# CCIG-Champalimaud/adell-mri

Hardware: AMD Instinct MI355X
Metric: volumes/sec 3D U-Net 128^3 2-ch seg (train step: fwd+loss+bwd+SGD) (higher is better)
Workload: dtype f32 (f16x3 split MFMA, fp32 accumulate); 1 GPU; BASELINE configs[1]: u-net-3d-resnet.yaml UNetPL, 2x128^3, batch 2/GPU, dice+focal, SGD-Nesterov; per_gpu_batch=2, parallelism=dp1, yaml=configs/u-net-3d-resnet.yaml, built_by=parse_config_unet -> get_segmentation_network('unet'), gradient_exchange=none (1 rank)

## Files before the change

### adell_mri_amd/_lib.py

```python
import ctypes
import os

_HERE = os.path.dirname(os.path.abspath(__file__))
LIB_PATH = os.environ.get("ADELL_HIP_LIBRARY") or os.path.join(_HERE, "libadellhip.so")

_lib = None

OK = 0
E_BADARG, E_UNSUPPORTED, E_HIP, E_NOMEM = -1, -2, -3, -4

ACT_IDS = {
    "identity": 0, "swish": 1, "silu": 1, "relu": 2, "leaky_relu": 3, "prelu": 4,
    "gelu": 5, "sigmoid": 6, "tanh": 7, "elu": 8,
}


class AdellHipError(RuntimeError):
    pass


class ConvDesc(ctypes.Structure):
    _fields_ = [(n, ctypes.c_int32) for n in (
        "N", "D", "H", "W", "C0", "C1", "Cout", "KD", "KH", "KW", "SD", "SH", "SW",
        "PD", "PH", "PW", "Do", "Ho", "Wo")]
# ... 213 lines not shown
    "adell_gather_nd": (_i, [_vp, _vp, _i, _vp, _vp, _vp, _i, _vp, _vp, _vp, _vp]),
    "adell_layernorm_rows_fwd": (_i, [_vp, _l, _i, _i, _l, _l, _vp, _vp, _f, _vp, _vp, _vp, _vp]),
    "adell_layernorm_rows_bwd_workspace": (_l, [_l, _i]),
    "adell_layernorm_rows_bwd": (_i, [_vp, _vp, _vp, _vp, _vp, _l, _i, _i, _l, _l, _vp, _l, _l,
                                      _vp, _vp, _vp, ctypes.c_size_t, _vp]),
    "adell_winattn_fwd": (_i, [_vp, _vp, _vp, _l, _l, _vp, _vp, _i, _l, _i, _i, _i, _i, _f, _f,
                               ctypes.c_ulong, ctypes.c_uint, _vp, _vp, _vp]),
    "adell_winattn_bwd": (_i, [_vp, _vp, _vp, _l, _l, _vp, _vp, _i, _vp, _vp, _vp, _l, _i, _i, _i,
                               _i, _f, _f, ctypes.c_ulong, ctypes.c_uint, _vp, _vp, _vp, _vp, _vp]),
    "adell_gemm_f32_workspace_floats": (_l, [_i, _i, _i]),
    "adell_gemm_f32": (_i, [_i, _i, _i, _vp, _l, _i, _vp, _l, _i, _vp, _l, _vp, _vp, _l, _vp, _vp]),
    "adell_absmax_f32": (_i, [_vp, _l, _vp, _vp]),
    "adell_gemm_f16x3_applicable": (_i, [_i, _i, _i, _vp, _l, _i, _vp, _l, _i]),
    "adell_gemm_f16x3_workspace_floats": (_l, [_i, _i, _i]),
    "adell_gemm_f16x3": (_i, [_i, _i, _i, _vp, _l, _i, _vp, _l, _i, _vp, _l, _vp, _vp, _l, _vp, _vp,
                              _vp, _vp]),
    "adell_gemm_f16x3_act": (_i, [_i, _i, _i, _vp, _l, _i, _vp, _l, _i, _vp, _l, _vp, _vp, _l, _vp,
                                  _vp, _vp, _i, _f, _vp, _vp, _vp]),
    "adell_optim_step": (_i, [_i, _vp, _vp, _vp, _vp, _l, _f, _f, _f, ctypes.POINTER(ctypes.c_float),
                              _vp]),
    "adell_seg_loss_workspace": (_l, [_i, _l, _i]),
    "adell_seg_loss_fwd": (_i, [_i, _vp, _vp, _vp, _i, _l, _i, _f, _f, _f, _f, _f, _f, _vp, _vp, _vp,
                                ctypes.c_size_t, _vp]),
    "adell_seg_loss_bwd": (_i, [_i, _vp, _vp, _vp, _i, _l, _i, _f, _f, _f, _f, _f, _f, _vp, _vp, _vp,
                                _vp]),
    "adell_channel_softmax_fwd": (_i, [_vp, _vp, _l, _i, _vp]),
    "adell_channel_softmax_bwd": (_i, [_vp, _vp, _vp, _l, _i, _vp]),
    "adell_channel_max_fwd": (_i, [_vp, _vp, _vp, _i, _l, _i, _vp]),
    "adell_channel_max_bwd": (_i, [_vp, _vp, _vp, _i, _l, _i, _vp]),
    "adell_debug_force_conv_cfg": (None, [_i]),
    "adell_set_tuning": (_i, [ctypes.c_char_p, _i]),
    "adell_rng_advance": (_i, [ctypes.c_uint32, _i, _vp]),
    "adell_get_tuning": (_i, [ctypes.c_char_p]),
}


def lib():
    global _lib
    if _lib is None:
        if not os.path.exists(LIB_PATH):
            raise AdellHipError(
                f"{LIB_PATH} not found: build it with `python -c 'import __graft_entry__ as g; "
                "g.build()'` (or `make -C adell_mri_amd/csrc`). adell_mri_amd has no fallback path."
            )
        import torch

        h = ctypes.CDLL(LIB_PATH)
        for name, (res, args) in SIGNATURES.items():
            fn = getattr(h, name)
            fn.restype = res
            fn.argtypes = args
        _lib = h
    return _lib


def check(rc):
    if rc != OK:
        msg = lib().adell_last_error().decode("utf-8", "replace")
        kind = {E_BADARG: "bad argument", E_UNSUPPORTED: "unsupported", E_HIP: "HIP error",
                E_NOMEM: "out of memory"}.get(rc, f"error {rc}")
        raise AdellHipError(f"libadellhip: {kind}: {msg}")
    return rc


class tuning:

# ... 17 lines not shown
```

### adell_mri_amd/csrc/api.hip

```cpp
#include "common.h"
#include <stdarg.h>

static thread_local char g_err[512] = "";

void adell_set_error(const char* fmt, ...) {
  va_list ap;
  va_start(ap, fmt);
  vsnprintf(g_err, sizeof(g_err), fmt, ap);
  va_end(ap);
}

extern "C" const char* adell_last_error(void) { return g_err; }
extern "C" int adell_abi_version(void) { return ADELL_ABI_VERSION; }

int adell_cu_count() {
  static const int cus = [] {
    int dev = 0, n = 0;
    if (hipGetDevice(&dev) != hipSuccess ||
        hipDeviceGetAttribute(&n, hipDeviceAttributeMultiprocessorCount, dev) != hipSuccess)
      n = 0;
    return n > 0 ? n : 256;
  }();
  return cus;
}

#include <stdlib.h>
#include <string.h>

static int adell_env_int(const char* name, int dflt) {
  const char* v = getenv(name);
  return v ? atoi(v) : dflt;
}
static int adell_env_set(const char* name) { return getenv(name) != nullptr; }

static AdellTuning adell_tuning_from_env() {
  AdellTuning t;
  t.igemm_nospec = adell_env_set("ADELL_IGEMM_NOSPEC");
  t.igemm_no8 = adell_env_set("ADELL_IGEMM_NO8");
  t.no_splitk = adell_env_set("ADELL_NO_SPLITK");
  t.wgrad_nozring = adell_env_set("ADELL_WGRAD_NOZRING");
  t.attn_nomfma = adell_env_set("ADELL_ATTN_NOMFMA");
  t.dw_nomfma = adell_env_int("ADELL_DW_NOMFMA", 0);
  t.dw_wgrad_nomfma = adell_env_int("ADELL_DW_WGRAD_NOMFMA", 0);
  t.wgrad_no16 = adell_env_int("ADELL_WGRAD_NO16", 0);
  t.igemm_no16 = adell_env_int("ADELL_IGEMM_NO16", 0);
  t.gemm_norows = adell_env_int("ADELL_GEMM_NOROWS", 0);
#ifdef ADELL_DEBUG
  t.igemm_dbg = adell_env_int("ADELL_IGEMM_DBG", 0);
  t.zr_dbg = adell_env_int("ADELL_ZR_DBG", 0);
#else
  t.igemm_dbg = 0;
  t.zr_dbg = 0;
#endif
  return t;
}
AdellTuning g_adell_tune = adell_tuning_from_env();
long g_adell_plan_epoch = 0;
extern "C" long adell_plan_epoch(void) { return g_adell_plan_epoch; }

static int* adell_tuning_slot(const char* name) {
  if (!name) return nullptr;
  if (!strcmp(name, "igemm_nospec")) return &g_adell_tune.igemm_nospec;
  if (!strcmp(name, "igemm_no8")) return &g_adell_tune.igemm_no8;
  if (!strcmp(name, "no_splitk")) return &g_adell_tune.no_splitk;
  if (!strcmp(name, "wgrad_nozring")) return &g_adell_tune.wgrad_nozring;
  if (!strcmp(name, "attn_nomfma")) return &g_adell_tune.attn_nomfma;
  if (!strcmp(name, "dw_nomfma")) return &g_adell_tune.dw_nomfma;
  if (!strcmp(name, "dw_wgrad_nomfma")) return &g_adell_tune.dw_wgrad_nomfma;
  if (!strcmp(name, "wgrad_no16")) return &g_adell_tune.wgrad_no16;
  if (!strcmp(name, "igemm_no16")) return &g_adell_tune.igemm_no16;
  if (!strcmp(name, "gemm_norows")) return &g_adell_tune.gemm_norows;
#ifdef ADELL_DEBUG
  if (!strcmp(name, "igemm_dbg")) return &g_adell_tune.igemm_dbg;
  if (!strcmp(name, "zr_dbg")) return &g_adell_tune.zr_dbg;
#endif
  return nullptr;
}

extern "C" int adell_set_tuning(const char* name, int value) {
  int* slot = adell_tuning_slot(name);
  if (!slot) {
    adell_set_error("adell_set_tuning: unknown switch '%s'", name ? name : "(null)");
    return ADELL_E_BADARG;
  }
  if (*slot != value) ++g_adell_plan_epoch;
  *slot = value;
  return ADELL_OK;
}

extern "C" int adell_get_tuning(const char* name) {
  int* slot = adell_tuning_slot(name);
  return slot ? *slot : -1;
}

int adell_rng_advance_norm_act(unsigned delta, int set, hipStream_t st);
int adell_rng_advance_tokens(unsigned delta, int set, hipStream_t st);
int adell_rng_advance_window(unsigned delta, int set, hipStream_t st);

extern "C" int adell_rng_advance(uint32_t delta, int set, void* stream) {
  hipStream_t st = (hipStream_t)stream;
  int rc = adell_rng_advance_norm_act(delta, set, st);
  if (rc == ADELL_OK) rc = adell_rng_advance_tokens(delta, set, st);
  if (rc == ADELL_OK) rc = adell_rng_advance_window(delta, set, st);
  if (rc != ADELL_OK) adell_set_error("adell_rng_advance: launch failed");
// ... 3 lines not shown
```

### adell_mri_amd/csrc/common.h

```cpp
#pragma once
#include <hip/hip_runtime.h>
#include <stdint.h>
#include <stdio.h>
#include "../../include/adell_hip.h"

typedef float f32x16 __attribute__((ext_vector_type(16)));
typedef float f32x4 __attribute__((ext_vector_type(4)));

#define ADELL_WAVE 64
#define ADELL_GLOBAL __attribute__((address_space(1)))

void adell_set_error(const char* fmt, ...);

struct AdellTuning {
  int igemm_nospec;
  int igemm_no8;
  int no_splitk;
  int wgrad_nozring;
  int attn_nomfma;
  int dw_nomfma;
  int dw_wgrad_nomfma;
  int wgrad_no16;
  int igemm_no16;
  int gemm_norows;
  int igemm_dbg, zr_dbg;
};
extern AdellTuning g_adell_tune;
extern long g_adell_plan_epoch;
#define ADELL_REQUIRE_ROWS(ptr, have, need, what)                                              \
  ADELL_REQUIRE((ptr) == nullptr || (long)(have) == (long)(need),                              \
                "%s: partial-sum buffer sized for %ld rows per item, the current launch plan "  \
                "writes %ld (query the matching *_ntiles again after adell_set_tuning)",        \
                what, (long)(have), (long)(need))
#ifdef ADELL_DEBUG
#define ADELL_DBG(bits) (bits)
#else
#define ADELL_DBG(bits) 0
#endif

#define ADELL_CHECK_HIP(expr)                                                  \
  do {                                                                         \
    hipError_t _e = (expr);                                                    \
    if (_e != hipSuccess) {                                                    \
      adell_set_error("%s:%d: %s -> %s", __FILE__, __LINE__, #expr,            \
                      hipGetErrorString(_e));                                  \
      return ADELL_E_HIP;                                                      \
    }                                                                          \
  } while (0)

#define ADELL_REQUIRE(cond, ...)                                               \
  do {                                                                         \
    if (!(cond)) {                                                             \
      adell_set_error(__VA_ARGS__);                                            \
      return ADELL_E_BADARG;                                                   \
    }                                                                          \
  } while (0)

// ... 121 lines not shown
```

### adell_mri_amd/csrc/norm_act.hip

```cpp
#include "common.h"

ADELL_RNG_STEP_DEFINE(norm_act)

__global__ __launch_bounds__(256) void adell_stats_finalize_kernel(
    const float* __restrict__ part, int N, int ntiles, int C, double count, float eps,
    int per_item, float* __restrict__ mean, float* __restrict__ rstd) {
  __shared__ double sh[8][32][2];
  const int cl = threadIdx.x & 31, sl = threadIdx.x >> 5;
  const int c = blockIdx.x * 32 + cl;
  const int nbeg = per_item ? blockIdx.y : 0, nend = per_item ? blockIdx.y + 1 : N;
  double s1 = 0.0, s2 = 0.0;
  if (c < C) {
    for (int n = nbeg; n < nend; ++n) {
      const float* p = part + ((size_t)n * ntiles * C + c) * 2;
      int t = sl;
      for (; t + 56 < ntiles; t += 64) {
        float2 v[8];
#pragma unroll
        for (int u = 0; u < 8; ++u)
          v[u] = *reinterpret_cast<const float2*>(p + (size_t)(t + 8 * u) * C * 2);
#pragma unroll
        for (int u = 0; u < 8; ++u) {
          s1 += (double)v[u].x;
          s2 += (double)v[u].y;
        }
      }
      for (; t < ntiles; t += 8) {
        const float2 v = *reinterpret_cast<const float2*>(p + (size_t)t * C * 2);
        s1 += (double)v.x;
        s2 += (double)v.y;
      }
    }
  }
  sh[sl][cl][0] = s1;
  sh[sl][cl][1] = s2;
  __syncthreads();
  if (sl == 0 && c < C) {
    double a = 0.0, b = 0.0;
#pragma unroll
    for (int k = 0; k < 8; ++k) {
      a += sh[k][cl][0];
      b += sh[k][cl][1];
    }
    const double cnt = per_item ? count : count * N;
    const double m = a / cnt;
    double var = b / cnt - m * m;
    if (var < 0.0) var = 0.0;
    const size_t o = per_item ? (size_t)blockIdx.y * C + c : (size_t)c;
    mean[o] = (float)m;
    rstd[o] = (float)(1.0 / sqrt(var + (double)eps));
  }
}

__global__ __launch_bounds__(256) void adell_stats_fold_kernel(const float* __restrict__ part,
                                                               int ntiles, int C, int Z,
                                                               float* __restrict__ out,
                                                               int pstride, int poff) {
  __shared__ double sh[8][32][2];
  const int cl = threadIdx.x & 31, sl = threadIdx.x >> 5;
  const int c = blockIdx.x * 32 + cl, n = blockIdx.y, z = blockIdx.z;
  const int t0 = z * 256;
  const int t1 = t0 + 256 < ntiles ? t0 + 256 : ntiles;
  double s1 = 0.0, s2 = 0.0;
  if (c < C) {
    const float* p = part + ((size_t)n * ntiles * pstride + poff + c) * 2;
    int t = t0 + sl;
    for (; t + 56 < t1; t += 64) {
      float2 v[8];
#pragma unroll
      for (int u = 0; u < 8; ++u)
        v[u] = *reinterpret_cast<const float2*>(p + (size_t)(t + 8 * u) * pstride * 2);
#pragma unroll
      for (int u = 0; u < 8; ++u) {
        s1 += (double)v[u].x;
        s2 += (double)v[u].y;
      }
    }
    for (; t < t1; t += 8) {
      const float2 v = *reinterpret_cast<const float2*>(p + (size_t)t * pstride * 2);
      s1 += (double)v.x;
      s2 += (double)v.y;
    }
  }
  sh[sl][cl][0] = s1;
  sh[sl][cl][1] = s2;
  __syncthreads();
  if (sl == 0 && c < C) {
    double a = 0.0, b = 0.0;
#pragma unroll
    for (int k = 0; k < 8; ++k) {
      a += sh[k][cl][0];
      b += sh[k][cl][1];
    }
    float* o = out + (((size_t)n * Z + z) * C + c) * 2;
    o[0] = (float)a;
    o[1] = (float)b;
  }
}

extern "C" long adell_stats_finalize_workspace(int N, int ntiles, int C) {
  if (ntiles <= 512) return 0;
  const long Z = (ntiles + 255) / 256;
  return (long)sizeof(float) * N * Z * C * 2;
}

extern "C" int adell_stats_finalize(const float* partials, int N, int ntiles, int C,
                                    long count, float eps, int per_item, float* mean,
                                    float* rstd, void* workspace, size_t workspace_bytes,
                                    void* stream) {
  ADELL_REQUIRE(partials && mean && rstd, "stats_finalize: null pointer");
  ADELL_REQUIRE(N > 0 && ntiles > 0 && C > 0 && count > 0, "stats_finalize: bad dims");
  hipStream_t st = (hipStream_t)stream;
  const long need = adell_stats_finalize_workspace(N, ntiles, C);
  if (need > 0) {
    ADELL_REQUIRE(workspace && (long)workspace_bytes >= need,
                  "stats_finalize: workspace too small");
    const int Z = (ntiles + 255) / 256;
    hipLaunchKernelGGL(adell_stats_fold_kernel, dim3(adell_cdiv(C, 32), N, Z), dim3(256), 0, st,
                       partials, ntiles, C, Z, (float*)workspace, C, 0);
    partials = (const float*)workspace;
    ntiles = Z;
  }
  hipLaunchKernelGGL(adell_stats_finalize_kernel, dim3(adell_cdiv(C, 32), per_item ? N : 1),
                     dim3(256), 0, st, partials, N, ntiles, C, (double)count, eps, per_item, mean,
                     rstd);
  ADELL_CHECK_HIP(hipGetLastError());
  return ADELL_OK;
}

__global__ __launch_bounds__(256) void adell_bn_running_update_kernel(
    const float* __restrict__ mean, const float* __restrict__ rstd, float* __restrict__ rmean,
    float* __restrict__ rvar, long long* __restrict__ nbt, int C, float unbias, float eps,
    float momentum) {
  long long t = nbt != nullptr ? nbt[0] + 1 : 0;
  const float mom = momentum >= 0.f ? momentum : 1.f / (float)t;
  __syncthreads();
  for (int c = threadIdx.x; c < C; c += 256) {
    const float r = rstd[c];
    const float var = (1.f / (r * r) - eps) * unbias;
    rmean[c] = rmean[c] * (1.f - mom) + mom * mean[c];
    rvar[c] = rvar[c] * (1.f - mom) + mom * var;
  }
  if (threadIdx.x == 0 && nbt != nullptr) nbt[0] = t;
}

extern "C" int adell_bn_running_update(const float* mean, const float* rstd, float* running_mean,
                                       float* running_var, long long* num_batches_tracked, int C,
                                       long count, float eps, float momentum, void* stream) {
  ADELL_REQUIRE(mean && rstd && running_mean && running_var && C > 0 && count > 0,
                "bn_running_update: bad arguments");
  ADELL_REQUIRE(momentum >= 0.f || num_batches_tracked != nullptr,
                "bn_running_update: the cumulative average needs num_batches_tracked");
  const float unbias = (float)((double)count / (double)(count > 1 ? count - 1 : 1));
  hipLaunchKernelGGL(adell_bn_running_update_kernel, dim3(1), dim3(256), 0, (hipStream_t)stream, mean,
                     rstd, running_mean, running_var, num_batches_tracked, C, unbias, eps, momentum);
// ... 575 lines not shown
    if (sl == 0 && c < C) {
      double A = 0.0, B = 0.0;
#pragma unroll
      for (int k = 0; k < 32; ++k) {
        A += sh[k][cl][0];
        B += sh[k][cl][1];
      }
      accA += A;
      accB += B;
      if (per_item) {
        const double g = gamma ? (double)gamma[c] : 1.0;
        c1[(size_t)n * C + c] = (float)(g * A / count);
        c2[(size_t)n * C + c] = (float)(g * B / count);
      }
    }
    __syncthreads();
  }
  if (sl == 0 && c < C) {
    if (!per_item) {
      const double g = gamma ? (double)gamma[c] : 1.0;
      c1[c] = (float)(g * accA / (count * N));
      c2[c] = (float)(g * accB / (count * N));
    }
    if (dgamma) dgamma[c] = (float)accB;
    if (dbeta) dbeta[c] = (float)accA;
  }
}

__global__ __launch_bounds__(256) void adell_na_bwd_finalize_item_kernel(
    const float* __restrict__ part, int ntiles, int C, double count,
    const float* __restrict__ gamma, float* __restrict__ c1, float* __restrict__ c2,
    int pstride, int poff) {
  __shared__ double sh[32][8][2];
  const int cl = threadIdx.x & 7, sl = threadIdx.x >> 3;
  const int c = blockIdx.x * 8 + cl, n = blockIdx.y;
  double a0 = 0.0, a1 = 0.0, b0 = 0.0, b1 = 0.0;
  if (c < C) {
    int t = sl;
    for (; t + 32 < ntiles; t += 64) {
      const float2 u =
          *reinterpret_cast<const float2*>(part + (((size_t)n * ntiles + t) * pstride + poff + c) * 2);
      const float2 v = *reinterpret_cast<const float2*>(
          part + (((size_t)n * ntiles + t + 32) * pstride + poff + c) * 2);
      a0 += (double)u.x; b0 += (double)u.y;
      a1 += (double)v.x; b1 += (double)v.y;
    }
    for (; t < ntiles; t += 32) {
      const float2 u =
          *reinterpret_cast<const float2*>(part + (((size_t)n * ntiles + t) * pstride + poff + c) * 2);
      a0 += (double)u.x; b0 += (double)u.y;
    }
  }
  sh[sl][cl][0] = a0 + a1;
  sh[sl][cl][1] = b0 + b1;
  __syncthreads();
  if (sl == 0 && c < C) {
    double A = 0.0, B = 0.0;
#pragma unroll
    for (int k = 0; k < 32; ++k) {
      A += sh[k][cl][0];
      B += sh[k][cl][1];
    }
    const double g = gamma ? (double)gamma[c] : 1.0;
    c1[(size_t)n * C + c] = (float)(g * A / count);
    c2[(size_t)n * C + c] = (float)(g * B / count);
  }
}

template <bool VEC>
__global__ __launch_bounds__(256) void adell_na_bwd_apply_kernel(NormActBwdArgs a) {
  constexpr int W = VEC ? 4 : 1;
  const long nw = a.total / W;
  const float keep_scale = a.drop_p > 0.f ? 1.0f / (1.0f - a.drop_p) : 1.0f;
  for (long i = blockIdx.x * (long)blockDim.x + threadIdx.x; i < nw;
       i += (long)gridDim.x * blockDim.x) {
    const long e = i * W;
    const int c = (int)(e % a.C);
    const long nidx = e / a.VC;
    bool keep[4];
    adell_na_keep4(a, e >> 2, keep);
    float xs[W], gs[W], out[W];
    if constexpr (VEC) {
      const float4 xv = *reinterpret_cast<const float4*>(a.x + e);
      const float4 gv = *reinterpret_cast<const float4*>(a.dout + e);
      xs[0] = xv.x; xs[1] = xv.y; xs[2] = xv.z; xs[3] = xv.w;
      gs[0] = gv.x; gs[1] = gv.y; gs[2] = gv.z; gs[3] = gv.w;
    } else {
      xs[0] = a.x[e];
      gs[0] = a.dout[e];
    }
#pragma unroll
    for (int j = 0; j < W; ++j) {
      const int cj = c + j;
      float dt, hn;
      adell_na_bwd_elem(a, xs[j], gs[j], nidx, cj, VEC ? keep[j] : keep[e & 3], keep_scale,
                        &dt, &hn);
      float r = dt;
      if (a.gamma) r *= a.gamma[cj];
      if (a.mean) {
// ... 122 lines not shown
  else
    hipLaunchKernelGGL(adell_na_bwd_apply_kernel<false>, dim3(adell_ew_blocks(nw)), dim3(256),
                       0, st, a);
}

static int adell_norm_act_bwd_impl(const adell_norm_act_desc* d, const float* x,
                                   const float* dout, const float* mean, const float* rstd,
                                   const float* gamma, const float* beta, const float* act_w,
                                   float* dx, float* dgamma, float* dbeta, void* workspace,
                                   size_t workspace_bytes, void* stream, const float* lr_g,
                                   const float* lr_w, int lr_co) {
  NormActBwdArgs a = {};
  int rc = adell_nab_fill(&a, d);
  if (rc != ADELL_OK) return rc;
  a.lr_g = lr_g; a.lr_w = lr_w; a.lr_co = lr_co;
  a.lr_shift = adell_ilog2(d->C) - 2;
  ADELL_REQUIRE(x && dout && dx, "norm_act_bwd: null pointer");
  ADELL_REQUIRE((mean == nullptr) == (rstd == nullptr), "norm_act_bwd: mean/rstd mismatch");
  hipStream_t st = (hipStream_t)stream;
  a.x = x; a.dout = dout; a.mean = mean; a.rstd = rstd; a.gamma = gamma; a.beta = beta;
  a.act_w = act_w; a.dx = dx;
  bool vec, fast;
  adell_na_bwd_route(a, d, &vec, &fast);
  if (mean || dgamma || dbeta) {
    ADELL_REQUIRE(workspace && (long)workspace_bytes >= adell_norm_act_bwd_workspace(d),
                  "norm_act_bwd: workspace too small");
    float* part = (float*)workspace;
    long ntmax = a.ntiles;
    if (adell_na_fast_blocks(d->V, d->C) > ntmax) ntmax = adell_na_fast_blocks(d->V, d->C);
    float* c1 = part + (size_t)d->N * ntmax * d->C * 2;
    float* c2 = c1 + (size_t)d->N * d->C;
    a.part = part; a.c1 = c1; a.c2 = c2;
    adell_na_bwd_partials_launch(a, d, fast, vec, st);
    if (d->stats_per_item && !dgamma && !dbeta && d->N <= 65535)
      hipLaunchKernelGGL(adell_na_bwd_finalize_item_kernel,
                         dim3(adell_cdiv(d->C, 8), (unsigned)d->N), dim3(256), 0, st,
                         (const float*)part, a.ntiles, d->C, (double)d->V, gamma, c1, c2, d->C, 0);
    else
      hipLaunchKernelGGL(adell_na_bwd_finalize_kernel, dim3(adell_cdiv(d->C, 32)), dim3(1024), 0,
                         st, (const float*)part, (int)d->N, a.ntiles, d->C, (double)d->V,
                         d->stats_per_item, gamma, c1, c2, dgamma, dbeta);
  }
  adell_na_bwd_apply_launch(a, d, fast, vec, st);
  ADELL_CHECK_HIP(hipGetLastError());
  return ADELL_OK;
}

struct NaConst {
  float m[4], r[4], g[4], b[4], p[4], c1[4], c2[4];
};

__device__ __forceinline__ void adell_na_consts(NaConst& k, const float* mean, const float* rstd,
                                                const float* gamma, const float* beta,
                                                const float* act_w, int act_w_n, float act_p,
                                                const float* c1, const float* c2, long sbase,
                                                int c, int cmask) {
#pragma unroll
  for (int j = 0; j < 4; ++j) {
    const int cj = (c + j) & cmask;
    k.m[j] = mean ? mean[sbase + cj] : 0.f;
    k.r[j] = rstd ? rstd[sbase + cj] : 1.f;
    k.g[j] = gamma ? gamma[cj] : 1.f;
    k.b[j] = beta ? beta[cj] : 0.f;
    k.p[j] = act_w ? act_w[act_w_n > 1 ? cj : 0] : act_p;
    k.c1[j] = c1 ? c1[sbase + cj] : 0.f;
    k.c2[j] = c2 ? c2[sbase + cj] : 0.f;
  }
}

struct NaLowRank {
  float w[4][4];
// ... 240 lines not shown
#pragma unroll
      for (int q = 0; q < 4; ++q) {
        const float hn = (xs[q] - k.m[q]) * k.r[q];
        o[q] = k.r[q] * (gs[q] - k.c1[q] - hn * k.c2[q]);
      }
      dxo[jj] = make_float4(o[0], o[1], o[2], o[3]);
    }
  }
}

extern "C" int adell_norm_act_bwd_from_dt(const adell_norm_act_desc* d, const float* x,
                                          const float* dt, const float* mean, const float* rstd,
                                          const float* partials, int ntiles, int pstride, int poff,
                                          float* dx, void* workspace, size_t workspace_bytes,
                                          void* stream) {
  NormActBwdArgs a = {};
  int rc = adell_nab_fill(&a, d);
  if (rc != ADELL_OK) return rc;
  ADELL_REQUIRE(x && dt && dx && mean && rstd && partials && workspace,
                "norm_act_bwd_from_dt: null pointer");
  ADELL_REQUIRE(d->stats_per_item == 1 && d->N <= 65535,
                "norm_act_bwd_from_dt: instance statistics only");
  ADELL_REQUIRE(ntiles > 0 && pstride >= d->C && poff >= 0 && poff + d->C <= pstride,
                "norm_act_bwd_from_dt: bad partials layout");
  ADELL_REQUIRE(adell_is_pow2(d->C) && d->C % 4 == 0 && d->C <= 1024 &&
                    (((uintptr_t)x | (uintptr_t)dt | (uintptr_t)dx) & 15) == 0,
                "norm_act_bwd_from_dt: needs a power-of-two C in 4..1024 and aligned tensors");
  const int Z = ntiles > 512 ? (ntiles + 255) / 256 : 0;
  ADELL_REQUIRE(workspace_bytes >= sizeof(float) * (2 + 2 * (size_t)Z) * d->N * d->C,
                "norm_act_bwd_from_dt: workspace too small");
  hipStream_t st = (hipStream_t)stream;
  float* c1 = (float*)workspace;
  float* c2 = c1 + (size_t)d->N * d->C;
  if (Z > 0) {
    float* folded = c2 + (size_t)d->N * d->C;
    hipLaunchKernelGGL(adell_stats_fold_kernel, dim3(adell_cdiv(d->C, 32), (unsigned)d->N, Z),
                       dim3(256), 0, st, partials, ntiles, d->C, Z, folded, pstride, poff);
    partials = folded;
    ntiles = Z;
    pstride = d->C;
    poff = 0;
  }
  hipLaunchKernelGGL(adell_na_bwd_finalize_item_kernel, dim3(adell_cdiv(d->C, 8), (unsigned)d->N),
                     dim3(256), 0, st, partials, ntiles, d->C, (double)d->V, (const float*)nullptr,
                     c1, c2, pstride, poff);
  a.x = x; a.dout = dt; a.mean = mean; a.rstd = rstd; a.c1 = c1; a.c2 = c2; a.dx = dx;
  long bx = ((a.VC >> 2) + 256 * ADELL_EW_UNROLL - 1) / (256 * ADELL_EW_UNROLL);
  if (bx > ADELL_EW_MAXBLOCKS) bx = ADELL_EW_MAXBLOCKS;
  if (bx < 1) bx = 1;
  hipLaunchKernelGGL(adell_na_bwd_apply_dt_kernel, dim3((unsigned)bx, (unsigned)d->N), dim3(256), 0,
                     st, a);
  ADELL_CHECK_HIP(hipGetLastError());
  return ADELL_OK;
}

__global__ __launch_bounds__(256) void adell_prelu_wgrad_partial_kernel(NormActBwdArgs a, int chunk) {
  __shared__ float sh[4][64];
  const long rows = a.total / a.C;
  const long r0 = (long)blockIdx.x * chunk;
  long r1 = r0 + chunk;
  if (r1 > rows) r1 = rows;
  const int cl = threadIdx.x & 63, vl = threadIdx.x >> 6;
  const int c = blockIdx.y * 64 + cl;
  const float keep_scale = a.drop_p > 0.f ? 1.0f / (1.0f - a.drop_p) : 1.0f;
  float s = 0.f;
  if (c < a.C) {
    for (long r = r0 + vl; r < r1; r += 4) {
      const long n = r / a.V;
      const long e = r * a.C + c;
      float h = a.x[e];
      if (a.mean) {
        const long si = n * a.stat_stride_n + c;
        h = (h - a.mean[si]) * a.rstd[si];
      }
      float t = h;
      if (a.gamma) t *= a.gamma[c];
      if (a.beta) t += a.beta[c];
      bool keep[4];
// ... 100 lines not shown
      for (; t < ntiles; t += 8) {
        const float2 v = *reinterpret_cast<const float2*>(p + (size_t)t * C * 2);
        s1 += (double)v.x;
        s2 += (double)v.y;
      }
    }
  }
  sh[sl][cl][0] = s1;
  sh[sl][cl][1] = s2;
  __syncthreads();
  if (sl == 0 && c < C) {
    double a = 0.0, b = 0.0;
#pragma unroll
    for (int k = 0; k < 8; ++k) {
      a += sh[k][cl][0];
      b += sh[k][cl][1];
    }
    rec[c] = a;
    rec[C + c] = b;
  }
  if (blockIdx.x == 0 && threadIdx.x == 0) rec[2 * C] = count * N;
}

extern "C" int adell_bn_stats_sums(const float* partials, int N, int ntiles, int C, long count,
                                   double* sums, void* workspace, size_t workspace_bytes,
                                   void* stream) {
  ADELL_REQUIRE(partials && sums, "bn_stats_sums: null pointer");
  ADELL_REQUIRE(N > 0 && ntiles > 0 && C > 0 && count > 0, "bn_stats_sums: bad dims");
  hipStream_t st = (hipStream_t)stream;
  const long need = adell_stats_finalize_workspace(N, ntiles, C);
  if (need > 0) {
    ADELL_REQUIRE(workspace && (long)workspace_bytes >= need, "bn_stats_sums: workspace too small");
    const int Z = (ntiles + 255) / 256;
    hipLaunchKernelGGL(adell_stats_fold_kernel, dim3(adell_cdiv(C, 32), N, Z), dim3(256), 0, st,
                       partials, ntiles, C, Z, (float*)workspace, C, 0);
    partials = (const float*)workspace;
    ntiles = Z;
  }
  hipLaunchKernelGGL(adell_bn_sums_kernel, dim3(adell_cdiv(C, 32)), dim3(256), 0, st, partials, N,
                     ntiles, C, (double)count, sums);
  ADELL_CHECK_HIP(hipGetLastError());
  return ADELL_OK;
}

__global__ __launch_bounds__(256) void adell_bn_stats_from_sums_kernel(
    const double* __restrict__ rec, int C, float eps, float* __restrict__ mean,
    float* __restrict__ rstd, float* __restrict__ rmean, float* __restrict__ rvar,
    long long* __restrict__ nbt, float momentum) {
  const double cnt = rec[2 * C];
  long long t = nbt != nullptr ? nbt[0] + 1 : 0;
  const float mom = momentum >= 0.f ? momentum : 1.f / (float)t;
  const float unbias = (float)(cnt / (cnt > 1.0 ? cnt - 1.0 : 1.0));
  __syncthreads();
  for (int c = threadIdx.x; c < C; c += 256) {
    const double m = rec[c] / cnt;
    double var = rec[C + c] / cnt - m * m;
    if (var < 0.0) var = 0.0;
    const float mf = (float)m, r = (float)(1.0 / sqrt(var + (double)eps));
    mean[c] = mf;
    rstd[c] = r;
    if (rmean != nullptr) {
      const float v = (1.f / (r * r) - eps) * unbias;
      rmean[c] = rmean[c] * (1.f - mom) + mom * mf;
      rvar[c] = rvar[c] * (1.f - mom) + mom * v;
    }
  }
  if (threadIdx.x == 0 && rmean != nullptr && nbt != nullptr) nbt[0] = t;
}
// ... 131 lines not shown
```

### include/adell_hip.h

```cpp
#ifndef ADELL_HIP_H
#define ADELL_HIP_H

#include <stddef.h>
#include <stdint.h>

#ifdef __cplusplus
extern "C" {
#endif
#if defined(__GNUC__) || defined(__clang__)
#pragma GCC visibility push(default)
#endif

#define ADELL_OK 0
#define ADELL_E_BADARG (-1)
#define ADELL_E_UNSUPPORTED (-2)
#define ADELL_E_HIP (-3)
#define ADELL_E_NOMEM (-4)

#define ADELL_ABI_VERSION 2

enum {
  ADELL_ACT_IDENTITY = 0,
  ADELL_ACT_SILU = 1,
  ADELL_ACT_RELU = 2,
// ... 486 lines not shown
                     long ldb, int b_kc, float* C, long ldc, const float* bias,
                     const float* residual, long ldr, const uint32_t* a_absmax,
                     const uint32_t* b_absmax, float* workspace, void* stream);
int adell_gemm_f16x3_act(int M, int N, int K, const float* A, long lda, int a_kc, const float* B,
                         long ldb, int b_kc, float* C, long ldc, const float* bias,
                         const float* residual, long ldr, const uint32_t* a_absmax,
                         const uint32_t* b_absmax, float* workspace, int act, float act_p,
                         float* act_out, const float* dact_in, void* stream);

long adell_seg_loss_workspace(int B, long V, int C);
int adell_seg_loss_fwd(int kind, const float* p, const float* t, const float* cw, int B, long V,
                       int C, float eps, float scale, float label_smoothing, float gamma,
                       float smooth, float w_pos, float* loss, float* sums, void* workspace,
                       size_t workspace_bytes, void* stream);
int adell_seg_loss_bwd(int kind, const float* p, const float* t, const float* cw, int B, long V,
                       int C, float eps, float scale, float label_smoothing, float gamma,
                       float smooth, float w_pos, const float* sums, const float* gout, float* dp,
                       void* stream);

int adell_channel_softmax_fwd(const float* x, float* y, long rows, int C, void* stream);
int adell_channel_softmax_bwd(const float* y, const float* dy, float* dx, long rows, int C,
                              void* stream);

int adell_channel_max_fwd(const float* x, float* out, int* arg, int N, long V, int C,
                          void* stream);
int adell_channel_max_bwd(const float* dout, const int* arg, float* dx, int N, long V, int C,
                          void* stream);

void adell_debug_force_conv_cfg(int cfg);

int adell_set_tuning(const char* name, int value);
int adell_rng_advance(uint32_t delta, int set, void* stream);
int adell_get_tuning(const char* name);

long adell_item_stats_workspace(int N, long per_item);
int adell_item_stats(const float* x, int N, long per_item, float* out, void* workspace,
                     size_t workspace_bytes, void* stream);
int adell_aug_intensity(const float* x, float* out, int N, long per_item, const float* params,
                        uint64_t seed, uint32_t rng_offset, void* stream);
int adell_affine_sample(const float* x, float* out, int N, int D, int H, int W, int C,
                        const float* theta, int linear, int pad_mode, void* stream);
int adell_axis_filter(const float* x, float* out, int N, int D, int H, int W, int C, int axis,
                      const float* taps, int radius, void* stream);
int adell_bias_field(const float* x, float* out, int N, int D, int H, int W, int C,
                     const float* coef, void* stream);
int adell_axis_lut_sample(const float* x, float* out, int N, int D, int H, int W, int C,
                          const float* lut, int linear, void* stream);
int adell_dw_mfma_ok(int N, int C, int D, int H, int W, int KD, int KH, int KW, const float* x,
                     const float* y);
int adell_dw_dense_ok(int N, int C, int D, int H, int W, int KD, int KH, int KW, const float* x,
                      const float* y);
int adell_dw_wgrad_mfma_ok(int N, int C, int D, int H, int W, int KD, int KH, int KW, const float* x,
                           const float* dy);

int adell_wgrad_zring_plan(int N, int D, int H, int W, int C0, int C1, int Cout, int KD, int KH,
                           int KW, int SD, int SH, int SW, int Do, int Ho, int Wo, int* plan);

int adell_rowscale_fwd(const float* gamma, const float* W, const float* b, float* W2, float* b2, int C,
                       int K, void* stream);
int adell_rowscale_bwd(const float* gamma, const float* W, const float* b, const float* dW2,
                       const float* db2, float* dgamma, float* dW, float* db, int C, int K,
                       void* stream);

int adell_window_ndhwc(const float* in, float* out, int N, int C, int Di, int Hi, int Wi, int Do, int Ho,
                       int Wo, int od, int oh, int ow, void* stream);

// ... 12 lines not shown
```

Measured before the change: 61.69 volumes/s.

## Fold stats finalize into fold kernel via last-block-done atomic tail

```diff
diff --git a/adell_mri_amd/_lib.py b/adell_mri_amd/_lib.py
--- a/adell_mri_amd/_lib.py
+++ b/adell_mri_amd/_lib.py
@@ -269,6 +269,7 @@
     "adell_set_tuning": (_i, [ctypes.c_char_p, _i]),
     "adell_rng_advance": (_i, [ctypes.c_uint32, _i, _vp]),
     "adell_get_tuning": (_i, [ctypes.c_char_p]),
+    "adell_fold_tail_counts": (_i, [ctypes.POINTER(ctypes.c_long), _i, _i]),
 }
 
 
diff --git a/adell_mri_amd/csrc/api.hip b/adell_mri_amd/csrc/api.hip
--- a/adell_mri_amd/csrc/api.hip
+++ b/adell_mri_amd/csrc/api.hip
@@ -45,6 +45,7 @@
   t.wgrad_no16 = adell_env_int("ADELL_WGRAD_NO16", 0);
   t.igemm_no16 = adell_env_int("ADELL_IGEMM_NO16", 0);
   t.gemm_norows = adell_env_int("ADELL_GEMM_NOROWS", 0);
+  t.no_fold_tails = adell_env_int("ADELL_NO_FOLD_TAILS", 0);
 #ifdef ADELL_DEBUG
   t.igemm_dbg = adell_env_int("ADELL_IGEMM_DBG", 0);
   t.zr_dbg = adell_env_int("ADELL_ZR_DBG", 0);
@@ -70,6 +71,7 @@
   if (!strcmp(name, "wgrad_no16")) return &g_adell_tune.wgrad_no16;
   if (!strcmp(name, "igemm_no16")) return &g_adell_tune.igemm_no16;
   if (!strcmp(name, "gemm_norows")) return &g_adell_tune.gemm_norows;
+  if (!strcmp(name, "no_fold_tails")) return &g_adell_tune.no_fold_tails;
 #ifdef ADELL_DEBUG
   if (!strcmp(name, "igemm_dbg")) return &g_adell_tune.igemm_dbg;
   if (!strcmp(name, "zr_dbg")) return &g_adell_tune.zr_dbg;
diff --git a/adell_mri_amd/csrc/common.h b/adell_mri_amd/csrc/common.h
--- a/adell_mri_amd/csrc/common.h
+++ b/adell_mri_amd/csrc/common.h
@@ -23,6 +23,7 @@
   int wgrad_no16;
   int igemm_no16;
   int gemm_norows;
+  int no_fold_tails;
   int igemm_dbg, zr_dbg;
 };
 extern AdellTuning g_adell_tune;
diff --git a/adell_mri_amd/csrc/norm_act.hip b/adell_mri_amd/csrc/norm_act.hip
--- a/adell_mri_amd/csrc/norm_act.hip
+++ b/adell_mri_amd/csrc/norm_act.hip
@@ -1,100 +1,238 @@
 #include "common.h"
+#include <atomic>
+#include <mutex>
 
 ADELL_RNG_STEP_DEFINE(norm_act)
+
+constexpr int kTailStreams = 16;
+constexpr int kTailSection = 512;
+constexpr int kTailGraphWords = 16384;
+static __device__ unsigned g_adell_tail_ring[kTailStreams * kTailSection + kTailGraphWords];
+
+static std::mutex g_tail_mutex;
+static hipStream_t g_tail_stream[kTailStreams];
+static int g_tail_streams_used = 0;
+static int g_tail_graph_cursor = 0;
+static std::atomic<long> g_tail_count[ADELL_FOLD_TAIL_COUNTS];
+
+static int adell_tail_slots(int groups, hipStream_t st) {
+  if (g_adell_tune.no_fold_tails || groups < 1 || groups > kTailSection) return -1;
+  hipStreamCaptureStatus cap = hipStreamCaptureStatusNone;
+  if (hipStreamIsCapturing(st, &cap) != hipSuccess) {
+    (void)hipGetLastError();
+    return -1;
+  }
+  std::lock_guard<std::mutex> lock(g_tail_mutex);
+  if (cap != hipStreamCaptureStatusNone) {
+    if (g_tail_graph_cursor + groups > kTailGraphWords) return -1;
+    const int slot = kTailStreams * kTailSection + g_tail_graph_cursor;
+    g_tail_graph_cursor += groups;
+    return slot;
+  }
+  for (int i = 0; i < g_tail_streams_used; ++i)
+    if (g_tail_stream[i] == st) return i * kTailSection;
+  if (g_tail_streams_used == kTailStreams) return -1;
+  g_tail_stream[g_tail_streams_used] = st;
+  return kTailSection * g_tail_streams_used++;
+}
+
+extern "C" int adell_fold_tail_counts(long* counts, int n, int reset) {
+  ADELL_REQUIRE(n >= 0 && n <= ADELL_FOLD_TAIL_COUNTS && (counts || n == 0),
+                "fold_tail_counts: at most %d counters", ADELL_FOLD_TAIL_COUNTS);
+  for (int i = 0; i < n; ++i) counts[i] = g_tail_count[i].load();
+  if (reset)
+    for (auto& c : g_tail_count) c.store(0);
+  return ADELL_OK;
+}
+
+__device__ __forceinline__ bool adell_tail_last_block(unsigned* counter, unsigned total) {
+  __shared__ unsigned s_ticket;
+  __threadfence();
+  __syncthreads();
+  if (threadIdx.x == 0)
+    s_ticket = __hip_atomic_fetch_add(counter, 1u, __ATOMIC_ACQ_REL, __HIP_MEMORY_SCOPE_AGENT);
+  __syncthreads();
+  if (s_ticket != total - 1) return false;
+  __threadfence();
+  if (threadIdx.x == 0) __hip_atomic_store(counter, 0u, __ATOMIC_RELAXED, __HIP_MEMORY_SCOPE_AGENT);
+  return true;
+}
+
+__device__ __forceinline__ void adell_stats_rows8(const float* p, size_t stride, int t0, int t1,
+                                                  int sl, double& s1, double& s2) {
+  int t = t0 + sl;
+  for (; t + 56 < t1; t += 64) {
+    float2 v[8];
+#pragma unroll
+    for (int u = 0; u < 8; ++u)
+      v[u] = *reinterpret_cast<const float2*>(p + (size_t)(t + 8 * u) * stride * 2);
+#pragma unroll
+    for (int u = 0; u < 8; ++u) {
+      s1 += (double)v[u].x;
+      s2 += (double)v[u].y;
+    }
+  }
+  for (; t < t1; t += 8) {
+    const float2 v = *reinterpret_cast<const float2*>(p + (size_t)t * stride * 2);
+    s1 += (double)v.x;
+    s2 += (double)v.y;
+  }
+}
+
+__device__ __forceinline__ void adell_stats_lanes8(const double (*sh)[32][2], int cl, double& a,
+                                                   double& b) {
+  a = 0.0;
+  b = 0.0;
+#pragma unroll
+  for (int k = 0; k < 8; ++k) {
+    a += sh[k][cl][0];
+    b += sh[k][cl][1];
+  }
+}
+
+__device__ __forceinline__ void adell_stats_finalize_block(const float* part, int N, int ntiles,
+                                                           int C, double count, float eps,
+                                                           int per_item, int cblock, int n0,
+                                                           float* mean, float* rstd,
+                                                           double (*sh)[32][2]) {
+  const int cl = threadIdx.x & 31, sl = threadIdx.x >> 5;
+  const int c = cblock * 32 + cl;
+  const int nbeg = per_item ? n0 : 0, nend = per_item ? n0 + 1 : N;
+  double s1 = 0.0, s2 = 0.0;
+  if (c < C) {
+    for (int n = nbeg; n < nend; ++n)
+      adell_stats_rows8(part + ((size_t)n * ntiles * C + c) * 2, (size_t)C, 0, ntiles, sl, s1, s2);
+  }
+  sh[sl][cl][0] = s1;
+  sh[sl][cl][1] = s2;
+  __syncthreads();
+  if (sl == 0 && c < C) {
+    double a, b;
+    adell_stats_lanes8(sh, cl, a, b);
+    const double cnt = per_item ? count : count * N;
+    const double m = a / cnt;
+    double var = b / cnt - m * m;
+    if (var < 0.0) var = 0.0;
+    const size_t o = per_item ? (size_t)n0 * C + c : (size_t)c;
+    mean[o] = (float)m;
+    rstd[o] = (float)(1.0 / sqrt(var + (double)eps));
+  }
+}
 
 __global__ __launch_bounds__(256) void adell_stats_finalize_kernel(
     const float* __restrict__ part, int N, int ntiles, int C, double count, float eps,
     int per_item, float* __restrict__ mean, float* __restrict__ rstd) {
   __shared__ double sh[8][32][2];
-  const int cl = threadIdx.x & 31, sl = threadIdx.x >> 5;
-  const int c = blockIdx.x * 32 + cl;
-  const int nbeg = per_item ? blockIdx.y : 0, nend = per_item ? blockIdx.y + 1 : N;
-  double s1 = 0.0, s2 = 0.0;
+  adell_stats_finalize_block(part, N, ntiles, C, count, eps, per_item, blockIdx.x, blockIdx.y, mean,
+                             rstd, sh);
+}
+
+__device__ __forceinline__ void adell_na_item_finalize_block(const float* part, int ntiles, int C,
+                                                             double count, const float* gamma,
+                                                             float* c1, float* c2, int pstride,
+                                                             int poff, int cblock, int n,
+                                                             double (*sh)[8][2]) {
+  const int cl = threadIdx.x & 7, sl = threadIdx.x >> 3;
+  const int c = cblock * 8 + cl;
+  double a0 = 0.0, a1 = 0.0, b0 = 0.0, b1 = 0.0;
   if (c < C) {
-    for (int n = nbeg; n < nend; ++n) {
-      const float* p = part + ((size_t)n * ntiles * C + c) * 2;
-      int t = sl;
-      for (; t + 56 < ntiles; t += 64) {
-        float2 v[8];
-#pragma unroll
-        for (int u = 0; u < 8; ++u)
-          v[u] = *reinterpret_cast<const float2*>(p + (size_t)(t + 8 * u) * C * 2);
-#pragma unroll
-        for (int u = 0; u < 8; ++u) {
-          s1 += (double)v[u].x;
-          s2 += (double)v[u].y;
-        }
-      }
-      for (; t < ntiles; t += 8) {
-        const float2 v = *reinterpret_cast<const float2*>(p + (size_t)t * C * 2);
-        s1 += (double)v.x;
-        s2 += (double)v.y;
-      }
-    }
-  }
-  sh[sl][cl][0] = s1;
-  sh[sl][cl][1] = s2;
+    int t = sl;
+    for (; t + 32 < ntiles; t += 64) {
+      const float2 u =
+          *reinterpret_cast<const float2*>(part + (((size_t)n * ntiles + t) * pstride + poff + c) * 2);
+      const float2 v = *reinterpret_cast<const float2*>(
+          part + (((size_t)n * ntiles + t + 32) * pstride + poff + c) * 2);
+      a0 += (double)u.x; b0 += (double)u.y;
+      a1 += (double)v.x; b1 += (double)v.y;
+    }
+    for (; t < ntiles; t += 32) {
+      const float2 u =
+          *reinterpret_cast<const float2*>(part + (((size_t)n * ntiles + t) * pstride + poff + c) * 2);
+      a0 += (double)u.x; b0 += (double)u.y;
+    }
+  }
+  sh[sl][cl][0] = a0 + a1;
+  sh[sl][cl][1] = b0 + b1;
   __syncthreads();
   if (sl == 0 && c < C) {
-    double a = 0.0, b = 0.0;
-#pragma unroll
-    for (int k = 0; k < 8; ++k) {
-      a += sh[k][cl][0];
-      b += sh[k][cl][1];
-    }
-    const double cnt = per_item ? count : count * N;
-    const double m = a / cnt;
-    double var = b / cnt - m * m;
-    if (var < 0.0) var = 0.0;
-    const size_t o = per_item ? (size_t)blockIdx.y * C + c : (size_t)c;
-    mean[o] = (float)m;
-    rstd[o] = (float)(1.0 / sqrt(var + (double)eps));
-  }
-}
-
+    double A = 0.0, B = 0.0;
+#pragma unroll
+    for (int k = 0; k < 32; ++k) {
+      A += sh[k][cl][0];
+      B += sh[k][cl][1];
+    }
+    const double g = gamma ? (double)gamma[c] : 1.0;
+    c1[(size_t)n * C + c] = (float)(g * A / count);
+    c2[(size_t)n * C + c] = (float)(g * B / count);
+  }
+}
+
+struct StatsFoldTail {
+  int slot;
+  double count;
+  float eps;
+  float* o1;
+  float* o2;
+};
+enum { kFoldTailNone = 0, kFoldTailFwd = 1, kFoldTailBwd = 2 };
+
+template <int TAIL>
 __global__ __launch_bounds__(256) void adell_stats_fold_kernel(const float* __restrict__ part,
                                                                int ntiles, int C, int Z,
-                                                               float* __restrict__ out,
-                                                               int pstride, int poff) {
+                                                               float* out, int pstride, int poff,
+                                                               StatsFoldTail tail) {
   __shared__ double sh[8][32][2];
   const int cl = threadIdx.x & 31, sl = threadIdx.x >> 5;
   const int c = blockIdx.x * 32 + cl, n = blockIdx.y, z = blockIdx.z;
   const int t0 = z * 256;
   const int t1 = t0 + 256 < ntiles ? t0 + 256 : ntiles;
   double s1 = 0.0, s2 = 0.0;
-  if (c < C) {
-    const float* p = part + ((size_t)n * ntiles * pstride + poff + c) * 2;
-    int t = t0 + sl;
-    for (; t + 56 < t1; t += 64) {
-      float2 v[8];
-#pragma unroll
-      for (int u = 0; u < 8; ++u)
-        v[u] = *reinterpret_cast<const float2*>(p + (size_t)(t + 8 * u) * pstride * 2);
-#pragma unroll
-      for (int u = 0; u < 8; ++u) {
-        s1 += (double)v[u].x;
-        s2 += (double)v[u].y;
-      }
-    }
-    for (; t < t1; t += 8) {
-      const float2 v = *reinterpret_cast<const float2*>(p + (size_t)t * pstride * 2);
-      s1 += (double)v.x;
-      s2 += (double)v.y;
-    }
-  }
+  if (c < C)
+    adell_stats_rows8(part + ((size_t)n * ntiles * pstride + poff + c) * 2, (size_t)pstride, t0, t1,
+                      sl, s1, s2);
   sh[sl][cl][0] = s1;
   sh[sl][cl][1] = s2;
   __syncthreads();
   if (sl == 0 && c < C) {
-    double a = 0.0, b = 0.0;
-#pragma unroll
-    for (int k = 0; k < 8; ++k) {
-      a += sh[k][cl][0];
-      b += sh[k][cl][1];
-    }
+    double a, b;
+    adell_stats_lanes8(sh, cl, a, b);
     float* o = out + (((size_t)n * Z + z) * C + c) * 2;
     o[0] = (float)a;
     o[1] = (float)b;
+  }
+  if constexpr (TAIL != kFoldTailNone) {
+    if (!adell_tail_last_block(&g_adell_tail_ring[tail.slot + n * gridDim.x + blockIdx.x], Z))
+      return;
+    if constexpr (TAIL == kFoldTailFwd) {
+      adell_stats_finalize_block(out, 0, Z, C, tail.count, tail.eps, 1, blockIdx.x, n, tail.o1,
+                                 tail.o2, sh);
+    } else {
+      for (int g = 0; g < 4; ++g) {
+        adell_na_item_finalize_block(out, Z, C, tail.count, nullptr, tail.o1, tail.o2, C, 0,
+                                     blockIdx.x * 4 + g, n,
+                                     reinterpret_cast<double(*)[8][2]>(&sh[0][0][0]));
+        __syncthreads();
+      }
+    }
+  }
+}
+
+static void adell_stats_fold_launch(int tailkind, const float* partials, int N, int ntiles, int C,
+                                    int Z, float* folded, int pstride, int poff, StatsFoldTail tail,
+                                    hipStream_t st) {
+  const dim3 grid(adell_cdiv(C, 32), N, Z);
+  if (tail.slot < 0) {
+    ++g_tail_count[ADELL_COUNT_STATS_FOLD];
+    hipLaunchKernelGGL(adell_stats_fold_kernel<kFoldTailNone>, grid, dim3(256), 0, st, partials,
+                       ntiles, C, Z, folded, pstride, poff, tail);
+  } else if (tailkind == kFoldTailFwd) {
+    ++g_tail_count[ADELL_COUNT_TAILS];
+    hipLaunchKernelGGL(adell_stats_fold_kernel<kFoldTailFwd>, grid, dim3(256), 0, st, partials,
+                       ntiles, C, Z, folded, pstride, poff, tail);
+  } else {
+    ++g_tail_count[ADELL_COUNT_TAILS];
+    hipLaunchKernelGGL(adell_stats_fold_kernel<kFoldTailBwd>, grid, dim3(256), 0, st, partials,
+                       ntiles, C, Z, folded, pstride, poff, tail);
   }
 }
 
@@ -116,11 +254,18 @@
     ADELL_REQUIRE(workspace && (long)workspace_bytes >= need,
                   "stats_finalize: workspace too small");
     const int Z = (ntiles + 255) / 256;
-    hipLaunchKernelGGL(adell_stats_fold_kernel, dim3(adell_cdiv(C, 32), N, Z), dim3(256), 0, st,
-                       partials, ntiles, C, Z, (float*)workspace, C, 0);
+    StatsFoldTail tail = {-1, (double)count, eps, mean, rstd};
+    if (per_item && N <= 65535) tail.slot = adell_tail_slots(adell_cdiv(C, 32) * N, st);
+    adell_stats_fold_launch(kFoldTailFwd, partials, N, ntiles, C, Z, (float*)workspace, C, 0, tail,
+                            st);
+    if (tail.slot >= 0) {
+      ADELL_CHECK_HIP(hipGetLastError());
+      return ADELL_OK;
+    }
     partials = (const float*)workspace;
     ntiles = Z;
   }
+  ++g_tail_count[ADELL_COUNT_STATS_FINALIZE];
   hipLaunchKernelGGL(adell_stats_finalize_kernel, dim3(adell_cdiv(C, 32), per_item ? N : 1),
                      dim3(256), 0, st, partials, N, ntiles, C, (double)count, eps, per_item, mean,
                      rstd);
@@ -762,39 +907,8 @@
     const float* __restrict__ gamma, float* __restrict__ c1, float* __restrict__ c2,
     int pstride, int poff) {
   __shared__ double sh[32][8][2];
-  const int cl = threadIdx.x & 7, sl = threadIdx.x >> 3;
-  const int c = blockIdx.x * 8 + cl, n = blockIdx.y;
-  double a0 = 0.0, a1 = 0.0, b0 = 0.0, b1 = 0.0;
-  if (c < C) {
-    int t = sl;
-    for (; t + 32 < ntiles; t += 64) {
-      const float2 u =
-          *reinterpret_cast<const float2*>(part + (((size_t)n * ntiles + t) * pstride + poff + c) * 2);
-      const float2 v = *reinterpret_cast<const float2*>(
-          part + (((size_t)n * ntiles + t + 32) * pstride + poff + c) * 2);
-      a0 += (double)u.x; b0 += (double)u.y;
-      a1 += (double)v.x; b1 += (double)v.y;
-    }
-    for (; t < ntiles; t += 32) {
-      const float2 u =
-          *reinterpret_cast<const float2*>(part + (((size_t)n * ntiles + t) * pstride + poff + c) * 2);
-      a0 += (double)u.x; b0 += (double)u.y;
-    }
-  }
-  sh[sl][cl][0] = a0 + a1;
-  sh[sl][cl][1] = b0 + b1;
-  __syncthreads();
-  if (sl == 0 && c < C) {
-    double A = 0.0, B = 0.0;
-#pragma unroll
-    for (int k = 0; k < 32; ++k) {
-      A += sh[k][cl][0];
-      B += sh[k][cl][1];
-    }
-    const double g = gamma ? (double)gamma[c] : 1.0;
-    c1[(size_t)n * C + c] = (float)(g * A / count);
-    c2[(size_t)n * C + c] = (float)(g * B / count);
-  }
+  adell_na_item_finalize_block(part, ntiles, C, count, gamma, c1, c2, pstride, poff, blockIdx.x,
+                               blockIdx.y, sh);
 }
 
 template <bool VEC>
@@ -983,11 +1097,12 @@
     float* c2 = c1 + (size_t)d->N * d->C;
     a.part = part; a.c1 = c1; a.c2 = c2;
     adell_na_bwd_partials_launch(a, d, fast, vec, st);
-    if (d->stats_per_item && !dgamma && !dbeta && d->N <= 65535)
+    if (d->stats_per_item && !dgamma && !dbeta && d->N <= 65535) {
+      ++g_tail_count[ADELL_COUNT_NA_BWD_FINALIZE_ITEM];
       hipLaunchKernelGGL(adell_na_bwd_finalize_item_kernel,
                          dim3(adell_cdiv(d->C, 8), (unsigned)d->N), dim3(256), 0, st,
                          (const float*)part, a.ntiles, d->C, (double)d->V, gamma, c1, c2, d->C, 0);
-    else
+    } else
       hipLaunchKernelGGL(adell_na_bwd_finalize_kernel, dim3(adell_cdiv(d->C, 32)), dim3(1024), 0,
                          st, (const float*)part, (int)d->N, a.ntiles, d->C, (double)d->V,
                          d->stats_per_item, gamma, c1, c2, dgamma, dbeta);
@@ -1294,18 +1409,25 @@
   hipStream_t st = (hipStream_t)stream;
   float* c1 = (float*)workspace;
   float* c2 = c1 + (size_t)d->N * d->C;
+  bool folded_done = false;
   if (Z > 0) {
     float* folded = c2 + (size_t)d->N * d->C;
-    hipLaunchKernelGGL(adell_stats_fold_kernel, dim3(adell_cdiv(d->C, 32), (unsigned)d->N, Z),
-                       dim3(256), 0, st, partials, ntiles, d->C, Z, folded, pstride, poff);
+    StatsFoldTail tail = {adell_tail_slots(adell_cdiv(d->C, 32) * (int)d->N, st), (double)d->V, 0.f,
+                          c1, c2};
+    adell_stats_fold_launch(kFoldTailBwd, partials, (int)d->N, ntiles, d->C, Z, folded, pstride,
+                            poff, tail, st);
+    folded_done = tail.slot >= 0;
     partials = folded;
     ntiles = Z;
     pstride = d->C;
     poff = 0;
   }
-  hipLaunchKernelGGL(adell_na_bwd_finalize_item_kernel, dim3(adell_cdiv(d->C, 8), (unsigned)d->N),
-                     dim3(256), 0, st, partials, ntiles, d->C, (double)d->V, (const float*)nullptr,
-                     c1, c2, pstride, poff);
+  if (!folded_done) {
+    ++g_tail_count[ADELL_COUNT_NA_BWD_FINALIZE_ITEM];
+    hipLaunchKernelGGL(adell_na_bwd_finalize_item_kernel,
+                       dim3(adell_cdiv(d->C, 8), (unsigned)d->N), dim3(256), 0, st, partials, ntiles,
+                       d->C, (double)d->V, (const float*)nullptr, c1, c2, pstride, poff);
+  }
   a.x = x; a.dout = dt; a.mean = mean; a.rstd = rstd; a.c1 = c1; a.c2 = c2; a.dx = dx;
   long bx = ((a.VC >> 2) + 256 * ADELL_EW_UNROLL - 1) / (256 * ADELL_EW_UNROLL);
   if (bx > ADELL_EW_MAXBLOCKS) bx = ADELL_EW_MAXBLOCKS;
@@ -1472,8 +1594,9 @@
   if (need > 0) {
     ADELL_REQUIRE(workspace && (long)workspace_bytes >= need, "bn_stats_sums: workspace too small");
     const int Z = (ntiles + 255) / 256;
-    hipLaunchKernelGGL(adell_stats_fold_kernel, dim3(adell_cdiv(C, 32), N, Z), dim3(256), 0, st,
-                       partials, ntiles, C, Z, (float*)workspace, C, 0);
+    hipLaunchKernelGGL(adell_stats_fold_kernel<kFoldTailNone>, dim3(adell_cdiv(C, 32), N, Z),
+                       dim3(256), 0, st, partials, ntiles, C, Z, (float*)workspace, C, 0,
+                       StatsFoldTail{-1, 0.0, 0.f, nullptr, nullptr});
     partials = (const float*)workspace;
     ntiles = Z;
   }
diff --git a/include/adell_hip.h b/include/adell_hip.h
--- a/include/adell_hip.h
+++ b/include/adell_hip.h
@@ -542,6 +542,12 @@
 int adell_set_tuning(const char* name, int value);
 int adell_rng_advance(uint32_t delta, int set, void* stream);
 int adell_get_tuning(const char* name);
+#define ADELL_COUNT_STATS_FOLD 0
+#define ADELL_COUNT_STATS_FINALIZE 1
+#define ADELL_COUNT_NA_BWD_FINALIZE_ITEM 2
+#define ADELL_COUNT_TAILS 3
+#define ADELL_FOLD_TAIL_COUNTS 4
+int adell_fold_tail_counts(long* counts, int n, int reset);
 
 long adell_item_stats_workspace(int N, long per_item);
 int adell_item_stats(const float* x, int N, long per_item, float* out, void* workspace,
```

Result: no change. 61.53 volumes/s (-0.3%).
